# xuankuzcr/Global-LVBA

Hardware: NVIDIA H100
Metric: LM iterations/sec (Jacobian+Hessian build + Schur solve) (higher is better)
Workload: dtype f64

## Files before the change

global-lvba_b200/csrc/factor_la.cuh:

```cuda
#pragma once
#include "envelope.cuh"

namespace lvba {

constexpr bool la_tile2(int P) { return P > 24; }
constexpr int la_tile2_threads(int P) { int s = 0; for (int m = 1; m <= P; ++m) s += (m + 1) / 2; return s; }
template <int P, bool kTile2>
struct LaCfg {
  static constexpr int kPairs = P * (P + 1) / 2;
  static constexpr int kOwners = kTile2 ? la_tile2_threads(P) : kPairs;
  static constexpr bool kRealloc = P > 24;
  static constexpr int kPairThreads = kRealloc ? ((kOwners + 127) / 128) * 128 : ((kOwners + 31) / 32) * 32;
  static constexpr int kLaThreads = 128;
  static constexpr int kThreads = kPairThreads + kLaThreads;
  static constexpr int kItemThreads = 96;
  static constexpr int kItems = (P - 1) * 6;
  static constexpr int kRounds = (kItems + kItemThreads - 1) / kItemThreads;
  static constexpr int S = 38;
  static constexpr int kPairRegs = kTile2 ? 200 : 104, kLaRegs = kTile2 ? 96 : 64;
  static constexpr int kDoubles = 6 * P * S + 2 * P * 36 + 2 * 36 + 36 + 2 * 36 + P * 6 + 48 + 40 + 48;
  static constexpr size_t kSmem = sizeof(double) * (size_t)kDoubles + sizeof(long long) * 64 + sizeof(int) * 64 + 32;
};

LVBA_DEV void cp_async16_zfill(void* smem, const void* gmem, bool valid) {
// ... 474 lines not shown
          const int i = (l21 >= 15) ? 5 : (l21 >= 10) ? 4 : (l21 >= 6) ? 3 : (l21 >= 3) ? 2 : (l21 >= 1) ? 1 : 0;
          const int j = l21 - i * (i + 1) / 2;
          double v = dg[i * 6 + j];
          double w = 0.0;
#pragma unroll
          for (int q = 0; q < 6; q += 2) { v -= l1[q * 6 + i] * T1[q * 6 + j]; w += l1[(q + 1) * 6 + i] * T1[(q + 1) * 6 + j]; }
          v -= w;
          if (lane < 21) sDu[i * 6 + j] = v;
          __syncwarp();
          invert_pivot(sDu, sK + nxt * 36, k + 1);
        }
        named_bar_sync(1, Cfg::kLaThreads);
        double zk[6];
#pragma unroll
        for (int q = 0; q < 6; ++q) zk[q] = sZ[c * 6 + q];
        if (lane < 6) z[6 * (long long)k + lane] = sZ[c * 6 + lane];
        __syncwarp();
        if (lane + 1 < P) {
          int slot = c + 1 + lane; if (slot >= P) slot -= P;
          const double2* lt2 = reinterpret_cast<const double2*>(Lc + slot * S);
          double acc[6];
#pragma unroll
          for (int x = 0; x < 6; ++x) acc[x] = sZ[slot * 6 + x];
#pragma unroll
          for (int q = 0; q < 6; ++q) {
            const double2 l0 = lt2[3 * q], l1 = lt2[3 * q + 1], l2 = lt2[3 * q + 2];
            acc[0] -= l0.x * zk[q]; acc[1] -= l0.y * zk[q]; acc[2] -= l1.x * zk[q]; acc[3] -= l1.y * zk[q]; acc[4] -= l2.x * zk[q]; acc[5] -= l2.y * zk[q];
          }
#pragma unroll
          for (int x = 0; x < 6; ++x) sZ[slot * 6 + x] = acc[x];
        }
        __syncwarp();
        if (lane < 6) sZ[c * 6 + lane] = (k + P < n) ? sZin[((k + P) & 7) * 6 + lane] : 0.0;
        if (J.progress && lane == 0 && (k & 3) == 3) progress_publish(J.progress, k + 1);
      } else {
        stream_row(k + 1);
        if (it < 5) {
          const int rl = k + 40, rz = k + P + 4;
          if (it == 0 && rl < n) {
            asm volatile("cp.async.ca.shared.global [%0], [%1], 4;" ::"r"((unsigned)__cvta_generic_to_shared(sLabF + (rl & 63))), "l"(e.first + rl));
          } else if (it == 1 && rl < n) {
            asm volatile("cp.async.ca.shared.global [%0], [%1], 8;" ::"r"((unsigned)__cvta_generic_to_shared(sLabRS + (rl & 63))), "l"(e.row_start + rl));
          } else if (it >= 2 && rz < n) {
            cp_async16_zfill(sZin + (rz & 7) * 6 + 2 * (it - 2), z + 6 * (long long)rz + 2 * (it - 2), true);
          }
        }
        double t[Cfg::kRounds][6];
#pragma unroll
        for (int rd = 0; rd < Cfg::kRounds; ++rd) {
          const int slot = slot_[rd], x = x_[rd];
          if (ent_[rd]) {
            const double* en = sEnter + (cur * P) * 36 + x * 6;
#pragma unroll
            for (int q = 0; q < 6; ++q) t[rd][q] = en[q];
          } else {
            const double* as = sA + cur * PS + slot * S;
#pragma unroll
            for (int q = 0; q < 6; ++q) t[rd][q] = as[q * 6 + x];
            const double* lr = Lc + slot * S;
#pragma unroll
            for (int r = 0; r < 6; ++r) {
              const double lv = lr[r * 6 + x];
              const double2 u0 = reinterpret_cast<const double2*>(T1 + r * 6)[0];
              const double2 u1 = reinterpret_cast<const double2*>(T1 + r * 6)[1];
              const double2 u2 = reinterpret_cast<const double2*>(T1 + r * 6)[2];
              t[rd][0] -= lv * u0.x; t[rd][1] -= lv * u0.y; t[rd][2] -= lv * u1.x; t[rd][3] -= lv * u1.y; t[rd][4] -= lv * u2.x; t[rd][5] -= lv * u2.y;
            }
// ... 204 lines not shown
```

global-lvba_b200/csrc/nd_kernels.cuh:

```cuda
#pragma once
#include "envelope.cuh"
#include "factor_la.cuh"
#include "nd_passes.h"

namespace lvba {

template <class F>
__global__ void __launch_bounds__(256) nd_pass_kernel(long long n, F f) {
  for (long long i = (long long)blockIdx.x * blockDim.x + threadIdx.x; i < n; i += (long long)gridDim.x * blockDim.x) f(i);
}

constexpr int kSpikeC = 4;
constexpr int kSpikeWarps = 4;
constexpr int kSpikeCols = kSpikeC * kSpikeWarps;
constexpr int kSpikeThreads = 32 * kSpikeWarps;
constexpr int kSpikeZStride = 26;
constexpr int kSpikeBS = 38;
constexpr int kSpikeBufs = 3;
constexpr size_t kSpikeSmem = sizeof(double) * (kSpikeBufs * 32 * kSpikeBS + kSpikeWarps * 33 * kSpikeZStride);
static_assert(kSpikeC == 4, "the reduce-scatter below is written for 24 values per lane");

__global__ void __launch_bounds__(kSpikeThreads)
nd_spike_kernel(const nd::SpikeJob* __restrict__ jobs) {
  extern __shared__ __align__(16) double smem_spike[];
  double* sRow = smem_spike;
  const nd::SpikeJob J = jobs[blockIdx.y];
  const EnvView e = J.e;
  const int c0 = blockIdx.x * kSpikeCols;
  if (c0 >= J.KS) return;
  const int tid = threadIdx.x, lane = tid & 31, warp = tid >> 5;
  const int cw = c0 + warp * kSpikeC;
  double* sZw = smem_spike + kSpikeBufs * 32 * kSpikeBS + warp * 33 * kSpikeZStride;
  const int n = e.n, n_stop = J.n_stop, KS = J.KS;
  if (lane < kSpikeZStride) sZw[32 * kSpikeZStride + lane] = 0.0;
  for (int o = tid; o < kSpikeBufs * 32 * kSpikeBS; o += kSpikeThreads) sRow[o] = 0.0;
  const int sb0 = tid / 18, sh = tid - sb0 * 18;
  const int og = (lane >> 2) * 3;
  const bool owner = (lane & 3) == 0;
  int ox[3], oc[3];
#pragma unroll
  for (int q = 0; q < 3; ++q) { ox[q] = (og + q) >> 2; oc[q] = (og + q) & 3; }
  __syncthreads();
  auto stage_row = [&](int k, int f, long long rs) {
    if (k >= n) return;
    const int jend = k < n_stop ? k : n_stop;
    const int nb = jend > f ? jend - f : 0;
    const double* src = J.L + rs * 36;
    double* dst = sRow + (k % kSpikeBufs) * (32 * kSpikeBS);
    if (tid < 126)
      for (int b = sb0; b < nb; b += 7) cp_async16_zfill(dst + b * kSpikeBS + 2 * sh, src + b * 36 + 2 * sh, true);
  };
  int f0 = e.first[0];
  int f1 = n > 1 ? e.first[1] : 0; long long rs1 = n > 1 ? e.row_start[1] : 0;
  int f2 = n > 2 ? e.first[2] : 0; long long rs2 = n > 2 ? e.row_start[2] : 0;
  int f3 = n > 3 ? e.first[3] : 0; long long rs3 = n > 3 ? e.row_start[3] : 0;
  double en[3];
// ... 43 lines not shown
          double a = l[0] * z[c];
#pragma unroll
          for (int y = 1; y < 6; ++y) a = fma(l[y], z[y * 4 + c], a);
          v[x * 4 + c] = a;
        }
      }
    }
    const bool b16 = lane & 16, b8 = lane & 8, b4 = lane & 4;
    double w12[12], w6[6], w3[3];
#pragma unroll
    for (int o = 0; o < 12; ++o) {
      const double send = b16 ? v[o] : v[o + 12];
      const double keep = b16 ? v[o + 12] : v[o];
      w12[o] = keep + __shfl_xor_sync(0xffffffffu, send, 16);
    }
#pragma unroll
    for (int o = 0; o < 6; ++o) {
      const double send = b8 ? w12[o] : w12[o + 6];
      const double keep = b8 ? w12[o + 6] : w12[o];
      w6[o] = keep + __shfl_xor_sync(0xffffffffu, send, 8);
    }
#pragma unroll
    for (int o = 0; o < 3; ++o) {
      const double send = b4 ? w6[o] : w6[o + 3];
      const double keep = b4 ? w6[o + 3] : w6[o];
      w3[o] = keep + __shfl_xor_sync(0xffffffffu, send, 4);
    }
#pragma unroll
    for (int o = 0; o < 3; ++o) {
      w3[o] += __shfl_xor_sync(0xffffffffu, w3[o], 2);
      w3[o] += __shfl_xor_sync(0xffffffffu, w3[o], 1);
    }
    __syncwarp();
    if (owner) {
#pragma unroll
      for (int q = 0; q < 3; ++q) {
        const double r = ecur[q] - w3[q];
        sZw[(k & 31) * kSpikeZStride + ox[q] * 4 + oc[q]] = r;
        if (cw + oc[q] < KS) J.Z[((long long)k * 6 + ox[q]) * KS + cw + oc[q]] = r;
      }
    }
    __syncwarp();
    f0 = f1; f1 = f2; f2 = f3; rs2 = rs3; f3 = f4; rs3 = rs4;
  }
}

constexpr int kSyrkTile = 64;
constexpr int kSyrkThreads = 64;
constexpr int kSyrkChunk = 4;
constexpr int kSyrkSplit = 8;
constexpr int kSyrkLd = kSyrkTile + 4;
constexpr int kSyrkTileDoubles = kSyrkChunk * 6 * kSyrkLd;
constexpr size_t kSyrkSmem = sizeof(double) * (5 * kSyrkTileDoubles + 2 * kSyrkChunk * 36 + 2 * kSyrkChunk * 6 + kSyrkChunk * 6);

__global__ void __launch_bounds__(kSyrkThreads)
nd_syrk_kernel(const nd::SyrkSeg* __restrict__ segs, int split) {
  constexpr int TS = kSyrkTile, RC = kSyrkChunk * 6, LD = kSyrkLd;
  extern __shared__ __align__(16) double smem_syrk[];
  double* sA = smem_syrk;
  double* sB = sA + 2 * kSyrkTileDoubles;
  double* sY = sB + 2 * kSyrkTileDoubles;
  double* sK = sY + kSyrkTileDoubles;
  double* sW = sK + 2 * kSyrkChunk * 36;
  double* sKw = sW + 2 * RC;
  const nd::SyrkSeg G = segs[blockIdx.z];
  int ti = 0, tj = 0;
  { int t = blockIdx.x; while ((ti + 1) * (ti + 2) / 2 <= t) ++ti; tj = t - ti * (ti + 1) / 2; }
  if (ti * TS >= G.KS) return;
  const int k0 = blockIdx.y * split;
  if (k0 >= G.rows) return;
  const int k1 = min(G.rows, k0 + split);
  const int tid = threadIdx.x, tx = tid & 7, ty = tid >> 3;
  const int KS = G.KS;
  auto prefetch = [&](int kc, int par) {
    const int nr = min(kSyrkChunk, k1 - kc) * 6;
    double* dA = sA + par * kSyrkTileDoubles;
    double* dB = sB + par * kSyrkTileDoubles;
    for (int o = tid; o < RC * (TS / 2); o += kSyrkThreads) {
      const int r = o / (TS / 2), a2 = (o - r * (TS / 2)) * 2;
      const double* zr = G.Z + ((long long)kc * 6 + (r < nr ? r : 0)) * KS;
      const bool va = r < nr && ti * TS + a2 < KS, vb = r < nr && tj * TS + a2 < KS;
      cp_async16_zfill(dA + r * LD + a2, va ? zr + ti * TS + a2 : G.Z, va);
      cp_async16_zfill(dB + r * LD + a2, vb ? zr + tj * TS + a2 : G.Z, vb);
    }
    for (int o = tid; o < kSyrkChunk * 18; o += kSyrkThreads) {
      const int bk = o / 18;
      const bool v = kc + bk < k1;
      cp_async16_zfill(sK + par * kSyrkChunk * 36 + 2 * o, v ? G.K + (long long)kc * 36 + 2 * o : G.K, v);
    }
    for (int o = tid; o < kSyrkChunk * 3; o += kSyrkThreads) {
      const int bk = o / 3;
      const bool v = kc + bk < k1;
      cp_async16_zfill(sW + par * RC + 2 * o, v ? G.w + (long long)kc * 6 + 2 * o : G.w, v);
    }
  };
  double acc[8][8];
#pragma unroll
  for (int i = 0; i < 8; ++i)
#pragma unroll
    for (int j = 0; j < 8; ++j) acc[i][j] = 0.0;
  double racc = 0.0;
  prefetch(k0, 0);
  asm volatile("cp.async.commit_group;" ::: "memory");
  int par = 0;
  for (int kc = k0; kc < k1; kc += kSyrkChunk, par ^= 1) {
    if (kc + kSyrkChunk < k1) prefetch(kc + kSyrkChunk, par ^ 1);
    asm volatile("cp.async.commit_group;" ::: "memory");
    asm volatile("cp.async.wait_group 1;" ::: "memory");
    __syncthreads();
    const double* cA = sA + par * kSyrkTileDoubles;
    const double* cB = sB + par * kSyrkTileDoubles;
    const double* cK = sK + par * kSyrkChunk * 36;
    for (int o = tid; o < RC * TS; o += kSyrkThreads) {
      const int r = o / TS, b = o - r * TS, bk = r / 6, x = r - bk * 6;
      const double* Kx = cK + bk * 36 + x * 6;
      double s = 0.0;
#pragma unroll
      for (int q = 0; q < 6; ++q) s += Kx[q] * cB[(bk * 6 + q) * LD + b];
      sY[r * LD + b] = s;
    }
    if (tj == 0 && tid < RC) {
      const int bk = tid / 6, x = tid - bk * 6;
      double s = 0.0;
#pragma unroll
      for (int q = 0; q < 6; ++q) s += cK[bk * 36 + x * 6 + q] * sW[par * RC + bk * 6 + q];
      sKw[tid] = s;
    }
    __syncthreads();
#pragma unroll 2
    for (int r = 0; r < RC; ++r) {
      double av[8], bv[8];
#pragma unroll
      for (int m = 0; m < 4; ++m) {
        const double2 a = *reinterpret_cast<const double2*>(cA + r * LD + 2 * ty + 16 * m);
        const double2 b = *reinterpret_cast<const double2*>(sY + r * LD + 2 * tx + 16 * m);
        av[2 * m] = a.x; av[2 * m + 1] = a.y; bv[2 * m] = b.x; bv[2 * m + 1] = b.y;
      }
#pragma unroll
      for (int i = 0; i < 8; ++i)
#pragma unroll
        for (int j = 0; j < 8; ++j) acc[i][j] = fma(av[i], bv[j], acc[i][j]);
    }
    if (tj == 0 && tid < TS) {
      double s = 0.0;
      for (int r = 0; r < RC; ++r) s += cA[r * LD + tid] * sKw[r];
      racc += s;
    }
    __syncthreads();
  }
#pragma unroll
  for (int i = 0; i < 8; ++i)
#pragma unroll
    for (int j = 0; j < 8; ++j) {
      const int ga = ti * TS + 2 * ty + 16 * (i >> 1) + (i & 1), gb = tj * TS + 2 * tx + 16 * (j >> 1) + (j & 1);
      const int bi = ga / 6, bj = gb / 6;
      if (bj <= bi && ga < KS && gb < KS) atomicAdd(&G.U[((long long)bi * (bi + 1) / 2 + bj) * 36 + (ga - 6 * bi) * 6 + (gb - 6 * bj)], -acc[i][j]);
    }
  if (tj == 0 && tid < TS && ti * TS + tid < KS) atomicAdd(&G.u[ti * TS + tid], -racc);
}

__global__ void __launch_bounds__(192)
nd_correct_apply_kernel(nd::Tables t, const int* __restrict__ ids, int stride) {
  __shared__ double sc[6];
  const nd::NodeDev v = t.nodes[ids[blockIdx.x / stride]];
  const int k = blockIdx.x % stride;
  if (k >= v.npiv) return;
  const int tid = threadIdx.x, lane = tid & 31, q = tid >> 5;
  const double* wv = (v.kind == 0 ? t.z : t.zs) + 6 * (long long)(v.r0 + k);
  const double* zr = t.Z + v.offZ + ((long long)k * 6 + q) * v.ks;
  const int na = 6 * v.wa;
  const double* xa = t.x + 6 * (long long)v.sa;
  const double* xc = t.x + 6 * (long long)v.sc;
  double s = 0.0;
  for (int col = lane; col < v.ks; col += 32) s += zr[col] * (col < na ? xa[col] : xc[col - na]);
  s = warp_sum(s);
  if (lane == 0) sc[q] = wv[q] - s;
  __syncthreads();
  if (tid < 6) {
    const double* K = t.dinv + (long long)(v.r0 + k) * 36 + tid * 6;
    double o = 0.0;
#pragma unroll
    for (int qq = 0; qq < 6; ++qq) o += K[qq] * sc[qq];
// ... 55 lines not shown
        }
        if (i == s) {
          double2* d2 = reinterpret_cast<double2*>(sD + r * 6);
          d2[0] = make_double2(t[0], t[1]); d2[1] = make_double2(t[2], t[3]); d2[2] = make_double2(t[4], t[5]);
        }
      }
      if (!idle) {
        named_bar_sync(2, kDenseColThreads + 32);
        named_bar_sync(3, kDenseColThreads + 32);
      }
      if (mine && i > s) {
        double lr[6] = {0, 0, 0, 0, 0, 0};
        const double2* k2 = reinterpret_cast<const double2*>(sK + par * 36);
#pragma unroll
        for (int q = 0; q < 6; ++q) {
          const double2 k0 = k2[3 * q], k1 = k2[3 * q + 1], kk2 = k2[3 * q + 2];
          lr[0] = fma(t[q], k0.x, lr[0]); lr[1] = fma(t[q], k0.y, lr[1]); lr[2] = fma(t[q], k1.x, lr[2]);
          lr[3] = fma(t[q], k1.y, lr[3]); lr[4] = fma(t[q], kk2.x, lr[4]); lr[5] = fma(t[q], kk2.y, lr[5]);
        }
        double* tt = sT + (par * kDenseMax + i) * kDenseS + r;
        double* lt = sL + (par * kDenseMax + i) * kDenseS + r;
        double2* g2 = reinterpret_cast<double2*>(J.L + ((long long)i * (i + 1) / 2 + s) * 36 + r * 6);
#pragma unroll
        for (int q = 0; q < 6; ++q) { tt[q * 6] = t[q]; lt[q * 6] = lr[q]; }
#pragma unroll
        for (int h = 0; h < 3; ++h) g2[h] = make_double2(lr[2 * h], lr[2 * h + 1]);
        double zs = 0.0;
#pragma unroll
        for (int q = 0; q < 6; ++q) { zs = fma(lr[q], sZ[s * 6 + q], zs); lrow[q] = lr[q]; }
        sZ[i * 6 + r] -= zs;
      }
      __syncthreads();
      if (idle) {
        if (ct - kDenseColThreads < 18)
          reinterpret_cast<double2*>(J.dinv + (long long)s * 36)[ct - kDenseColThreads] = reinterpret_cast<const double2*>(sK + par * 36)[ct - kDenseColThreads];
        if (J.progress && ct == kDenseColThreads + 32 && (s & 3) == 3) progress_publish(J.progress, s + 1);
      }
    }
  } else if (tid >= kDenseInvWarp) {
    const int lane = tid - kDenseInvWarp;
    int bad = 0;
    __syncthreads();
    for (int s = 0; s < n; ++s) {
      named_bar_sync(2, kDenseColThreads + 32);
      double* Kp = sK + (s & 1) * 36;
      sym6_block_inverse_warp(sD, Kp, sInv, lane);
      __syncwarp();
      if (!isfinite((Kp[0] + Kp[35]) + (Kp[18] + Kp[13]))) bad = 1;
      named_bar_sync(3, kDenseColThreads + 32);
      __syncthreads();
    }
    if (bad && lane == 0) J.status[0] = 1;
  } else {
    const unsigned short tm = tmap[tid];
    const int i = tm & 0xff, j = tm >> 8;
    const bool live = tm != 0xffff && i < n;
    double G[36];
    if (live) {
      const double2* src = reinterpret_cast<const double2*>(J.L + ((long long)i * (i + 1) / 2 + j) * 36);
#pragma unroll
      for (int q = 0; q < 18; ++q) { const double2 v = src[q]; G[2 * q] = v.x; G[2 * q + 1] = v.y; }
    } else {
#pragma unroll
      for (int q = 0; q < 36; ++q) G[q] = 0.0;
    }
    auto publish = [&](int c) {
      double2* d2 = reinterpret_cast<double2*>(sC + ((c & 1) * kDenseMax + i) * kDenseS);
#pragma unroll
      for (int q = 0; q < 18; ++q) d2[q] = make_double2(G[2 * q], G[2 * q + 1]);
    };
    if (live && j <= 1) publish(j);
    __syncthreads();
    for (int s = 0; s < n; ++s) {
      if (s >= 1 && live && j >= s + 1) {
        const int par = (s - 1) & 1;
        const double2* l2 = reinterpret_cast<const double2*>(sL + (par * kDenseMax + i) * kDenseS);
        const double2* t2 = reinterpret_cast<const double2*>(sT + (par * kDenseMax + j) * kDenseS);
#pragma unroll
        for (int q = 0; q < 6; ++q) {
          const double2 t0 = t2[3 * q], t1 = t2[3 * q + 1], t2v = t2[3 * q + 2];
#pragma unroll
          for (int xp = 0; xp < 3; ++xp) {
            const double2 lv = l2[3 * q + xp];
            const double l0 = -lv.x, l1 = -lv.y;
            double* g0 = G + (2 * xp) * 6;
            double* g1 = G + (2 * xp + 1) * 6;
            g0[0] = fma(l0, t0.x, g0[0]); g0[1] = fma(l0, t0.y, g0[1]); g0[2] = fma(l0, t1.x, g0[2]);
            g0[3] = fma(l0, t1.y, g0[3]); g0[4] = fma(l0, t2v.x, g0[4]); g0[5] = fma(l0, t2v.y, g0[5]);
            g1[0] = fma(l1, t0.x, g1[0]); g1[1] = fma(l1, t0.y, g1[1]); g1[2] = fma(l1, t1.x, g1[2]);
            g1[3] = fma(l1, t1.y, g1[3]); g1[4] = fma(l1, t2v.x, g1[4]); g1[5] = fma(l1, t2v.y, g1[5]);
          }
        }
        if (j == s + 1) publish(s + 1);
      }
      __syncthreads();
    }
  }
  __syncthreads();
  for (int o = tid; o < n * 6; o += kDenseThreads) J.z[o] = sZ[o];
  if (J.progress) {
    __syncthreads();
    if (tid == 0) progress_publish(J.progress, n);
  }
}

inline std::vector<unsigned short> dense_thread_map() {
  struct B { int i, j; };
  std::vector<B> v;
  for (int i = 0; i < kDenseMax; ++i) for (int j = 0; j <= i; ++j) v.push_back(B{i, j});
  std::stable_sort(v.begin(), v.end(), [](const B& a, const B& b) {
    const int ka[4] = {a.i / 8, a.j / 4, a.i, a.j}, kb[4] = {b.i / 8, b.j / 4, b.i, b.j};
    for (int q = 0; q < 4; ++q) if (ka[q] != kb[q]) return ka[q] < kb[q];
    return false;
  });
  std::vector<unsigned short> m((size_t)kDensePairThreads, (unsigned short)0xffff);
  for (size_t t = 0; t < v.size(); ++t) m[t] = (unsigned short)(v[t].i | (v[t].j << 8));
  return m;
}

}
```

global-lvba_b200/csrc/nd_passes.h:

```cpp
#pragma once
#include <math.h>
#include <stdint.h>

#include "env_types.h"
#include "nd_plan.h"

#if defined(__CUDACC__)
#define LVBA_NHD __host__ __device__ __forceinline__
#else
#define LVBA_NHD inline
#endif

namespace lvba {
namespace nd {

struct NodeDev {
  int kind, r0, npiv, ntrail, sa, wa, sc, wc, left, right, ks, nE, nb, zrows;
  long long offU, offu, offZ, offE, offT, offW, offw;
};
inline NodeDev to_dev(const Node& v) {
  return NodeDev{v.kind, v.r0, v.npiv, v.ntrail, v.sa, v.wa, v.sc, v.wc, v.left, v.right, v.ks, v.nE, v.nb, v.zrows,
                 v.offU, v.offu, v.offZ, v.offE, v.offT, v.offW, v.offw};
}

struct SpikeJob {
  EnvView e;
  const double* L;
  int n_stop;
  const double* E;
  int nE;
  double* Z;
  int KS;
  const int* progress = nullptr;
};
struct SyrkSeg {
  const double* Z;
  const double* K;
  const double* w;
  int rows;
  int KS;
  double* U;
  double* u;
};

struct Tables {
  int n;
  const int* first;
  const long long* row_start;
  const NodeDev* nodes;
  const double* H;
  const double* dadd;
  double* L;
  double* z;
  double* zs;
  double* dinv;
  double* x;
  double* U; double* u; double* Z; double* E; double* T; double* W; double* w;
  double* Hw; double* daddw;
  int* prog = nullptr;
};

LVBA_NHD void tri_dec(long long t, int& a, int& b) {
  long long i = (long long)((sqrt(8.0 * (double)t + 1.0) - 1.0) * 0.5);
  while ((i + 1) * (i + 2) / 2 <= t) ++i;
  while (i * (i + 1) / 2 > t) --i;
  a = (int)i;
  b = (int)(t - i * (i + 1) / 2);
}
LVBA_NHD long long tri_off(int i, int j) { return ((long long)i * (i + 1) / 2 + j) * 36; }
LVBA_NHD double mat_elem(const Tables& t, int r, int c, int x, int y) {
  if (c < t.first[r]) return 0.0;
  const double* b = t.H + (t.row_start[r] + (c - t.first[r])) * 36;
  if (r == c) {
    const double v = (x >= y) ? b[x * 6 + y] : b[y * 6 + x];
    return (x == y) ? v + t.dadd[6 * r + x] : v;
  }
  return b[x * 6 + y];
}
LVBA_NHD double upd_elem(const double* U, int i, int j, int x, int y) {
  return (i >= j) ? U[tri_off(i, j) + x * 6 + y] : U[tri_off(j, i) + y * 6 + x];
}

struct AddDiagF {
  Tables t;
  LVBA_NHD void operator()(int64_t i) const {
    const int r = (int)(i / 6), a = (int)(i % 6);
    t.L[(t.row_start[r] + (r - t.first[r])) * 36 + a * 7] += t.dadd[i];
  }
};

struct LeafEF {
  Tables t; const int* ids; long long stride;
// ... 219 lines not shown

struct DenseViewArrays {
  const int* zeros;
  const long long* tri;
  const int* last_by_w;
};

inline void build_level_jobs(const Plan& P, const Tables& t, const int* first_rel, const long long* rs_adj, const int* last_rel,
                             long long nblocks, const DenseViewArrays& dv, int* status, std::vector<LevelJobs>& out, int my_rank = 0) {
  out.assign(P.levels.size(), LevelJobs());
  for (size_t lv = 0; lv < P.levels.size(); ++lv) {
    LevelJobs& J = out[lv];
    for (int id : P.levels[lv])
      if (P.nodes[id].owner < 0 || P.nodes[id].owner == my_rank) J.ids.push_back(id);
    for (int id : J.ids) {
      const Node& v = P.nodes[id];
      EnvView e;
      double* Lp;
      double* zp;
      if (v.kind == 0) {
        e = EnvView{v.npiv + v.ntrail, first_rel + v.r0, rs_adj + v.r0, last_rel + v.r0, nblocks};
        Lp = t.L; zp = t.z + 6 * (long long)v.r0;
        for (int r = v.r0; r < v.r0 + v.npiv + v.ntrail; ++r) J.max_col = std::max(J.max_col, r - v.r0 - P.first_rel[r]);
      } else {
        e = EnvView{v.npiv, dv.zeros, dv.tri, dv.last_by_w + v.npiv * 32, (long long)v.npiv * (v.npiv + 1) / 2};
        Lp = t.T + v.offT; zp = t.zs + 6 * (long long)v.r0;
        J.max_col = std::max(J.max_col, v.npiv - 1);
      }
      J.factor.push_back(FactorJob{e, Lp, t.dinv + 36 * (long long)v.r0, zp, v.npiv,
                                   v.ntrail ? t.W + v.offW : nullptr, v.ntrail ? t.w + v.offw : nullptr, status + id,
                                   (t.prog && v.ks > 0) ? t.prog + id : nullptr});
      J.back.push_back(BacksolveJob{e, Lp, t.x + 6 * (long long)v.r0, v.npiv});
      if (v.ks > 0) {
        J.spike.push_back(SpikeJob{e, Lp, v.npiv, t.E + v.offE, v.kind == 0 ? v.nE : v.npiv, t.Z + v.offZ, v.ks, t.prog ? t.prog + id : nullptr});
        J.syrk.push_back(SyrkSeg{t.Z + v.offZ, t.dinv + 36 * (long long)v.r0, zp, v.npiv, v.ks, t.U + v.offU, t.u + v.offu});
        J.max_ks = std::max(J.max_ks, v.ks);
      }
      J.max_rows = std::max(J.max_rows, v.npiv);
      J.corr_stride = std::max(J.corr_stride, v.npiv);
      if (v.kind == 1) J.asm_stride = std::max(J.asm_stride, sep_items(v));
    }
  }
}

struct LevelDev {
  const int* ids; int n_ids;
  const FactorJob* factor; int n_factor;
  const SpikeJob* spike; int n_spike;
  const SyrkSeg* syrk; int n_syrk;
  const BacksolveJob* back; int n_back;
  long long asm_stride; int corr_stride; int max_ks, max_rows, max_col;
};

template <class Exec>
inline void run_up_local(Exec& ex, const Plan& P, const Tables& t, const LevelDev* lv, int n_levels, long long nblocks,
                         long long leaf_e, long long leaf_fin, const RegionDev* reg) {
  ex.copy(t.L, t.H, nblocks * 36);
  if (t.prog) ex.pass((long long)P.nodes.size(), ZeroProgF{t.prog});
  ex.pass((long long)6 * t.n, AddDiagF{t});
  ex.zero(t.U, P.sizeU);
  const LevelDev& L0 = lv[0];
  if (L0.n_spike) ex.pass((long long)L0.n_ids * leaf_e, LeafEF{t, L0.ids, leaf_e});
  ex.factor(L0.factor, L0.n_factor, L0.max_col);
  if (L0.n_spike) {
    ex.spike(L0.spike, L0.n_spike, L0.max_ks, P.max_zrows_leaf);
    ex.syrk(L0.syrk, L0.n_syrk, L0.max_ks, L0.max_rows);
  }
  ex.pass((long long)L0.n_ids * leaf_fin, LeafFinalF{t, L0.ids, leaf_fin});
  const int n_local = P.n_ranks > 1 ? P.local_levels : n_levels;
  for (int l = 1; l < n_local; ++l) {
    const LevelDev& J = lv[l];
    if (J.n_ids == 0) continue;
    ex.pass((long long)J.n_ids * J.asm_stride, SepAssembleF{t, J.ids, J.asm_stride});
    ex.factor_dense(J.factor, J.n_factor, J.max_col);
    if (J.n_spike) {
      ex.spike(J.spike, J.n_spike, J.max_ks, J.max_rows);
      ex.syrk(J.syrk, J.n_syrk, J.max_ks, J.max_rows);
    }
  }
  if (P.n_ranks > 1 && reg) ex.pass(reg->slotH + (long long)reg->slot_rows * 6, PackF{t, *reg});
}

template <class Exec>
inline void run_top_down(Exec& ex, const Plan& P, const Tables& t, const LevelDev* lv, int n_levels, const RegionDev* reg) {
  if (P.n_ranks > 1 && reg) {
    ex.pass((long long)reg->n_ranks * (reg->slotH + (long long)reg->slot_rows * 6), UnpackF{t, *reg});
    for (int l = P.local_levels; l < n_levels; ++l) {
      const LevelDev& J = lv[l];
      if (J.n_ids == 0) continue;
      ex.pass((long long)J.n_ids * J.asm_stride, SepAssembleF{t, J.ids, J.asm_stride});
      ex.factor_dense(J.factor, J.n_factor, J.max_col);
// ... 24 lines not shown
```

global-lvba_b200/csrc/nd_solver.cuh:

```cuda
#pragma once
#include <functional>

#include "nd_kernels.cuh"

namespace lvba {

struct NdDevice {
  nd::Plan plan;
  bool ready = false;
  int chunks = 0;
  DevBuf<int> d_first_rel, d_last_rel, d_zeros, d_last_by_w, d_ids;
  DevBuf<long long> d_rs_adj, d_tri;
  DevBuf<nd::NodeDev> d_nodes;
  DevBuf<int> d_sep_row0, d_sep_rows;
  nd::RegionDev reg{};
  int n_ranks = 1, my_rank = 0;
  DevBuf<double> xchg;
  DevBuf<unsigned short> d_dense_map;
  DevBuf<int> d_prog;
  DevBuf<double> zs, U, u, Z, E, T, W, w;
  DevBuf<FactorJob> d_factor;
  DevBuf<nd::SpikeJob> d_spike;
  DevBuf<nd::SyrkSeg> d_syrk;
  DevBuf<BacksolveJob> d_back;
  std::vector<nd::LevelDev> lv;
  nd::Tables tab{};
  long long leaf_e = 1, leaf_fin = 1;
  const double* key_H = nullptr; const double* key_dadd = nullptr; const double* key_x = nullptr; const double* key_z = nullptr;
  cudaGraph_t graph = nullptr;
  cudaGraphExec_t graph_exec = nullptr;
  bool use_graph = true;
  int64_t launches_per_solve = 0;

  ~NdDevice() { drop_graph(); }
  void drop_graph() {
    if (graph_exec) { cudaGraphExecDestroy(graph_exec); graph_exec = nullptr; }
    if (graph) { cudaGraphDestroy(graph); graph = nullptr; }
  }

  static int default_chunks(int n, int max_col) {
    if (n < 768) return 0;
    const long long want = (long long)n / (3LL * max_col + 30);
    int best = 0;
    for (int p = 4; p <= 256 && p <= want; p *= 2) best = p;
    return best;
  }

  int prepare(int n, const std::vector<int>& first, const std::vector<int>& last, const std::vector<long long>& row_start, int max_col,
              int p_want, cudaStream_t s, int n_ranks_ = 1, int my_rank_ = 0) {
    ready = false; chunks = 0;
    drop_graph();
    key_H = key_dadd = key_x = key_z = nullptr;
    n_ranks = n_ranks_; my_rank = my_rank_;
    if (n_ranks > 1) p_want = std::max(n_ranks, ((p_want + n_ranks - 1) / n_ranks) * n_ranks);
    if (p_want < 2) return LVBA_OK;
    const int p = nd::choose_chunks(n, first.data(), last.data(), row_start.data(), max_col, p_want, plan, n_ranks);
    if (p < 2) return LVBA_OK;
    if (n_ranks > 1) {
      for (int r = 0; r < n_ranks; ++r)
        if (plan.rank_row_end[r] - plan.rank_row_begin[r] < max_col + 1) return LVBA_OK;
    }
    {
      const char* g = getenv("LVBA_ND_GRAPH");
      use_graph = !(g && g[0] == '0');
    }
    int64_t dummy = 0;
    LVBA_TRY(d_first_rel.upload(plan.first_rel, s, &dummy));
    LVBA_TRY(d_last_rel.upload(plan.last_rel, s, &dummy));
    LVBA_TRY(d_rs_adj.upload(plan.rs_adj, s, &dummy));
    std::vector<int> zeros(32, 0), last_by_w(32 * 32, 0);
    std::vector<long long> tri(33, 0);
    for (int i = 0; i < 33; ++i) tri[i] = (long long)i * (i + 1) / 2;
    for (int w_ = 0; w_ < 32; ++w_) for (int i = 0; i < 32; ++i) last_by_w[w_ * 32 + i] = w_ - 1;
    LVBA_TRY(d_zeros.upload(zeros, s, &dummy));
    LVBA_TRY(d_last_by_w.upload(last_by_w, s, &dummy));
    LVBA_TRY(d_tri.upload(tri, s, &dummy));
    std::vector<nd::NodeDev> nodes;
    for (const nd::Node& v : plan.nodes) nodes.push_back(nd::to_dev(v));
    LVBA_TRY(d_nodes.upload(nodes, s, &dummy));
    const std::vector<unsigned short> dmap = dense_thread_map();
    LVBA_TRY(d_dense_map.upload(dmap, s, &dummy));
    LVBA_TRY(zs.alloc((size_t)n * 6));
    LVBA_TRY(U.alloc((size_t)std::max<long long>(plan.sizeU, 1))); LVBA_TRY(u.alloc((size_t)std::max<long long>(plan.sizeu, 1)));
    LVBA_TRY(Z.alloc((size_t)std::max<long long>(plan.sizeZ, 1))); LVBA_TRY(E.alloc((size_t)std::max<long long>(plan.sizeE, 1)));
    LVBA_TRY(T.alloc((size_t)std::max<long long>(plan.sizeT, 1))); LVBA_TRY(W.alloc((size_t)std::max<long long>(plan.sizeW, 1)));
    LVBA_TRY(w.alloc((size_t)std::max<long long>(plan.sizew, 1)));
    if (n_ranks > 1) {
      std::vector<int> s0((size_t)n_ranks, -1), sr((size_t)n_ranks, 0);
      for (int r = 0; r + 1 < n_ranks; ++r) { s0[r] = plan.sep_start[(r + 1) * plan.q]; sr[r] = plan.sep_width[(r + 1) * plan.q]; }
      LVBA_TRY(d_sep_row0.upload(s0, s, &dummy)); LVBA_TRY(d_sep_rows.upload(sr, s, &dummy));
      reg = nd::RegionDev{n_ranks, my_rank, plan.slot_rows, plan.max_col, plan.region0, plan.slot, plan.slotU, plan.slotu, plan.slotH,
                          d_sep_row0.p, d_sep_rows.p};
      long long mx = 0;
      for (int r = 0; r < n_ranks; ++r) {
        const int b = plan.rank_row_begin[r], e2 = std::min(n, b + max_col);
        mx = std::max(mx, (row_start[e2] - row_start[b]) * 36);
      }
      LVBA_TRY(xchg.alloc((size_t)std::max<long long>(mx, 1)));
    }
    LVBA_TRY(d_prog.alloc(plan.nodes.size()));
    LVBA_CUDA(cudaFuncSetAttribute(nd_spike_kernel, cudaFuncAttributeMaxDynamicSharedMemorySize, (int)kSpikeSmem));
    LVBA_CUDA(cudaFuncSetAttribute(nd_syrk_kernel, cudaFuncAttributeMaxDynamicSharedMemorySize, (int)kSyrkSmem));
    LVBA_CUDA(cudaFuncSetAttribute(nd_dense_factor_kernel, cudaFuncAttributeMaxDynamicSharedMemorySize, (int)kDenseSmem));
    LVBA_CUDA(cudaStreamSynchronize(s));
    leaf_e = nd::leaf_e_stride(plan); leaf_fin = nd::leaf_final_stride(plan);
    chunks = p; ready = true;
    return LVBA_OK;
  }

  int build_tables(const EnvView& genv, const double* H, const double* dadd, double* L, double* dinv, double* z, double* x,
                   int* status, cudaStream_t s) {
    if (key_H == H && key_dadd == dadd && key_x == x && key_z == z && !lv.empty()) return LVBA_OK;
    drop_graph();
    tab = nd::Tables{};
    tab.n = plan.n; tab.first = genv.first; tab.row_start = genv.row_start; tab.nodes = d_nodes.p;
    tab.H = H; tab.dadd = dadd; tab.L = L; tab.z = z; tab.zs = zs.p; tab.dinv = dinv; tab.x = x;
    tab.U = U.p; tab.u = U.p; tab.Z = Z.p; tab.E = E.p; tab.T = T.p; tab.W = W.p; tab.w = w.p;
    tab.Hw = n_ranks > 1 ? const_cast<double*>(H) : nullptr;
    tab.daddw = n_ranks > 1 ? const_cast<double*>(dadd) : nullptr;
    tab.prog = d_prog.p;
    std::vector<nd::LevelJobs> jobs;
    nd::DenseViewArrays dv{d_zeros.p, d_tri.p, d_last_by_w.p};
    nd::build_level_jobs(plan, tab, d_first_rel.p, d_rs_adj.p, d_last_rel.p, genv.nblocks, dv, status + 1, jobs, my_rank);
    std::vector<int> ids; std::vector<FactorJob> fj; std::vector<nd::SpikeJob> sj; std::vector<nd::SyrkSeg> yj; std::vector<BacksolveJob> bj;
    struct Off { size_t ids, f, s, y, b; };
    std::vector<Off> off;
    for (auto& J : jobs) {
      off.push_back(Off{ids.size(), fj.size(), sj.size(), yj.size(), bj.size()});
      ids.insert(ids.end(), J.ids.begin(), J.ids.end());
      fj.insert(fj.end(), J.factor.begin(), J.factor.end());
      sj.insert(sj.end(), J.spike.begin(), J.spike.end());
      yj.insert(yj.end(), J.syrk.begin(), J.syrk.end());
      bj.insert(bj.end(), J.back.begin(), J.back.end());
    }
    LVBA_TRY(d_ids.upload(ids, s)); LVBA_TRY(d_factor.upload(fj, s)); LVBA_TRY(d_back.upload(bj, s));
    if (!sj.empty()) { LVBA_TRY(d_spike.upload(sj, s)); LVBA_TRY(d_syrk.upload(yj, s)); }
    LVBA_CUDA(cudaStreamSynchronize(s));
    lv.clear();
    for (size_t l = 0; l < jobs.size(); ++l) {
      const auto& J = jobs[l];
      lv.push_back(nd::LevelDev{d_ids.p + off[l].ids, (int)J.ids.size(), d_factor.p + off[l].f, (int)J.factor.size(),
                                d_spike.p + off[l].s, (int)J.spike.size(), d_syrk.p + off[l].y, (int)J.syrk.size(),
                                d_back.p + off[l].b, (int)J.back.size(), J.asm_stride, J.corr_stride, J.max_ks, J.max_rows, J.max_col});
    }
    key_H = H; key_dadd = dadd; key_x = x; key_z = z;
    return LVBA_OK;
  }
};

struct NdCudaExec {
  cudaStream_t s;
  std::function<int(int, int, const FactorJob*)> factor_fn;
  std::function<void(int, const BacksolveJob*)> back_fn;
// ... 3 lines not shown
  template <class F> void pass(long long n, const F& f) {
    if (n <= 0) return;
    const int grid = (int)std::min<long long>((n + 255) / 256, kNumSMs * 8);
    nd_pass_kernel<<<grid, 256, 0, s>>>(n, f);
    ++launches;
  }
  void copy(double* dst, const double* src, long long n) { cudaMemcpyAsync(dst, src, (size_t)n * sizeof(double), cudaMemcpyDeviceToDevice, s); }
  void zero(double* p, long long n) { if (n > 0) cudaMemsetAsync(p, 0, (size_t)n * sizeof(double), s); }
  void factor(const FactorJob* jobs, int n, int max_col) {
    if (n <= 0) return;
    const int r = factor_fn(max_col, n, jobs);
    if (r != LVBA_OK) rc = r;
  }
  void factor_dense(const FactorJob* jobs, int n, int max_col) {
    if (n <= 0) return;
    nd_dense_factor_kernel<<<n, kDenseThreads, kDenseSmem, s>>>(jobs, dense_map);
    ++launches;
  }
  void spike(const nd::SpikeJob* jobs, int n, int max_ks, int) {
    if (n <= 0 || max_ks <= 0) return;
    cudaLaunchConfig_t cfg = {};
    cfg.gridDim = dim3((max_ks + kSpikeCols - 1) / kSpikeCols, n); cfg.blockDim = dim3(kSpikeThreads); cfg.dynamicSmemBytes = kSpikeSmem; cfg.stream = s;
    cudaLaunchAttribute at[1];
    at[0].id = cudaLaunchAttributeProgrammaticStreamSerialization;
    at[0].val.programmaticStreamSerializationAllowed = 1;
    cfg.attrs = at; cfg.numAttrs = 1;
    const cudaError_t e = cudaLaunchKernelEx(&cfg, nd_spike_kernel, jobs);
    if (e != cudaSuccess) rc = fail(LVBA_ERR_CUDA, "cudaLaunchKernelEx(nd_spike_kernel): %s", cudaGetErrorString(e));
    ++launches;
  }
  void syrk(const nd::SyrkSeg* segs, int n, int max_ks, int max_rows) {
    if (n <= 0 || max_ks <= 0) return;
    const int nt1 = (max_ks + kSyrkTile - 1) / kSyrkTile, nt = nt1 * (nt1 + 1) / 2;
    nd_syrk_kernel<<<dim3(nt, (max_rows + kSyrkSplit - 1) / kSyrkSplit, n), kSyrkThreads, kSyrkSmem, s>>>(segs, kSyrkSplit);
    ++launches;
  }
  void correct_apply(const nd::Tables& t, const int* ids, int n_ids, int stride) {
    if (n_ids <= 0 || stride <= 0) return;
    nd_correct_apply_kernel<<<n_ids * stride, 192, 0, s>>>(t, ids, stride);
    ++launches;
  }
  void backsolve(const BacksolveJob* jobs, int n) {
    if (n <= 0) return;
    back_fn(n, jobs);
    ++launches;
  }
};

}
```

Before: 330.5.

## Overlap spike and SYRK kernels via per-column-group progress counters and PDL

The spike kernel now triggers programmatic dependent launch and publishes per-column-group row progress counters, and the SYRK kernel is launched with PDL and polls these counters (plus the factor progress) so it can start consuming Z rows before the spike finishes. SYRK single-buffers the B tile to save shared memory and handles partial chunks. The dense factor writes z rows incrementally instead of at the end, and the heuristic for the number of chunks changes to scale with sqrt(n). This aims to hide the serial gap between kernels, at the cost of spin-polling, more progress memory, and the risk of deadlock if the blocks are not co-resident.

```diff
diff --git a/global-lvba_b200/csrc/factor_la.cuh b/global-lvba_b200/csrc/factor_la.cuh
--- a/global-lvba_b200/csrc/factor_la.cuh
+++ b/global-lvba_b200/csrc/factor_la.cuh
@@ -530,7 +530,7 @@
         }
         __syncwarp();
         if (lane < 6) sZ[c * 6 + lane] = (k + P < n) ? sZin[((k + P) & 7) * 6 + lane] : 0.0;
-        if (J.progress && lane == 0 && (k & 3) == 3) progress_publish(J.progress, k + 1);
+        if (J.progress && lane == 0 && (k & 3) == 3 && k + 1 < n_stop) progress_publish(J.progress, k + 1);
       } else {
         stream_row(k + 1);
         if (it < 5) {
diff --git a/global-lvba_b200/csrc/nd_kernels.cuh b/global-lvba_b200/csrc/nd_kernels.cuh
--- a/global-lvba_b200/csrc/nd_kernels.cuh
+++ b/global-lvba_b200/csrc/nd_kernels.cuh
@@ -18,10 +18,12 @@
 constexpr int kSpikeBS = 38;
 constexpr int kSpikeBufs = 3;
 constexpr size_t kSpikeSmem = sizeof(double) * (kSpikeBufs * 32 * kSpikeBS + kSpikeWarps * 33 * kSpikeZStride);
+constexpr int kSpikePublish = 4;
 static_assert(kSpikeC == 4, "the reduce-scatter below is written for 24 values per lane");
 
 __global__ void __launch_bounds__(kSpikeThreads)
 nd_spike_kernel(const nd::SpikeJob* __restrict__ jobs) {
+  pdl_launch_dependents();
   extern __shared__ __align__(16) double smem_spike[];
   double* sRow = smem_spike;
   const nd::SpikeJob J = jobs[blockIdx.y];
@@ -131,6 +133,7 @@
       w3[o] += __shfl_xor_sync(0xffffffffu, w3[o], 1);
     }
     __syncwarp();
+    if (J.zprog && tid == 32 && k > 0 && k % kSpikePublish == 0) progress_publish(J.zprog + blockIdx.x, k);
     if (owner) {
 #pragma unroll
       for (int q = 0; q < 3; ++q) {
@@ -141,6 +144,11 @@
     }
     __syncwarp();
     f0 = f1; f1 = f2; f2 = f3; rs2 = rs3; f3 = f4; rs3 = rs4;
+  }
+  if (J.zprog) {
+    wait_row(n);
+    __syncthreads();
+    if (tid == 0) progress_publish(J.zprog + blockIdx.x, n);
   }
 }
 
@@ -150,7 +158,11 @@
 constexpr int kSyrkSplit = 8;
 constexpr int kSyrkLd = kSyrkTile + 4;
 constexpr int kSyrkTileDoubles = kSyrkChunk * 6 * kSyrkLd;
-constexpr size_t kSyrkSmem = sizeof(double) * (5 * kSyrkTileDoubles + 2 * kSyrkChunk * 36 + 2 * kSyrkChunk * 6 + kSyrkChunk * 6);
+constexpr size_t kSyrkSmem = sizeof(double) * (4 * kSyrkTileDoubles + 2 * kSyrkChunk * 36 + 2 * kSyrkChunk * 6 + kSyrkChunk * 6);
+constexpr int kSyrkTileGroups = kSyrkTile / kSpikeCols;
+static_assert(kSyrkTile % kSpikeCols == 0 && kSyrkChunk % kSpikePublish == 0 && kSyrkSplit % kSyrkChunk == 0,
+              "a chunk of the SYRK must end where the spike publishes");
+static_assert(2 * kSyrkTileGroups + 1 <= kSyrkThreads, "one polling thread per counter");
 
 __global__ void __launch_bounds__(kSyrkThreads)
 nd_syrk_kernel(const nd::SyrkSeg* __restrict__ segs, int split) {
@@ -158,29 +170,43 @@
   extern __shared__ __align__(16) double smem_syrk[];
   double* sA = smem_syrk;
   double* sB = sA + 2 * kSyrkTileDoubles;
-  double* sY = sB + 2 * kSyrkTileDoubles;
+  double* sY = sB + kSyrkTileDoubles;
   double* sK = sY + kSyrkTileDoubles;
   double* sW = sK + 2 * kSyrkChunk * 36;
   double* sKw = sW + 2 * RC;
-  const nd::SyrkSeg G = segs[blockIdx.z];
+  const nd::SyrkSeg G = segs[blockIdx.y];
   int ti = 0, tj = 0;
   { int t = blockIdx.x; while ((ti + 1) * (ti + 2) / 2 <= t) ++ti; tj = t - ti * (ti + 1) / 2; }
   if (ti * TS >= G.KS) return;
-  const int k0 = blockIdx.y * split;
+  const int k0 = blockIdx.z * split;
   if (k0 >= G.rows) return;
   const int k1 = min(G.rows, k0 + split);
   const int tid = threadIdx.x, tx = tid & 7, ty = tid >> 3;
   const int KS = G.KS;
+  const int* poll = nullptr;
+  if (G.zprog) {
+    if (tid < 2 * kSyrkTileGroups) {
+      const int g = (tid < kSyrkTileGroups ? ti : tj) * kSyrkTileGroups + tid % kSyrkTileGroups;
+      if (g * kSpikeCols < KS) poll = G.zprog + g;
+    } else if (tid == 2 * kSyrkTileGroups) {
+      poll = G.fprog;
+    }
+  }
+  auto need = [&](int r) { return poll == G.fprog ? min(r + 1, G.rows) : r; };
+  auto wait_rows = [&](int r) {
+    if (poll) { const int v = need(r); while (progress_read(poll) < v) __nanosleep(64); }
+  };
+  auto rows_ready = [&](int r) { return !poll || progress_read(poll) >= need(r); };
+  auto wait_spike_done = [&]() {
+    if (poll && tid < 2 * kSyrkTileGroups) while (progress_read(poll) < G.zdone) __nanosleep(64);
+  };
   auto prefetch = [&](int kc, int par) {
     const int nr = min(kSyrkChunk, k1 - kc) * 6;
     double* dA = sA + par * kSyrkTileDoubles;
-    double* dB = sB + par * kSyrkTileDoubles;
     for (int o = tid; o < RC * (TS / 2); o += kSyrkThreads) {
       const int r = o / (TS / 2), a2 = (o - r * (TS / 2)) * 2;
-      const double* zr = G.Z + ((long long)kc * 6 + (r < nr ? r : 0)) * KS;
-      const bool va = r < nr && ti * TS + a2 < KS, vb = r < nr && tj * TS + a2 < KS;
-      cp_async16_zfill(dA + r * LD + a2, va ? zr + ti * TS + a2 : G.Z, va);
-      cp_async16_zfill(dB + r * LD + a2, vb ? zr + tj * TS + a2 : G.Z, vb);
+      const bool va = r < nr && ti * TS + a2 < KS;
+      cp_async16_zfill(dA + r * LD + a2, va ? G.Z + ((long long)kc * 6 + r) * KS + ti * TS + a2 : G.Z, va);
     }
     for (int o = tid; o < kSyrkChunk * 18; o += kSyrkThreads) {
       const int bk = o / 18;
@@ -193,24 +219,38 @@
       cp_async16_zfill(sW + par * RC + 2 * o, v ? G.w + (long long)kc * 6 + 2 * o : G.w, v);
     }
   };
+  auto prefetch_col = [&](int kc) {
+    const int nr = min(kSyrkChunk, k1 - kc) * 6;
+    for (int o = tid; o < RC * (TS / 2); o += kSyrkThreads) {
+      const int r = o / (TS / 2), a2 = (o - r * (TS / 2)) * 2;
+      const bool vb = r < nr && tj * TS + a2 < KS;
+      cp_async16_zfill(sB + r * LD + a2, vb ? G.Z + ((long long)kc * 6 + r) * KS + tj * TS + a2 : G.Z, vb);
+    }
+  };
   double acc[8][8];
 #pragma unroll
   for (int i = 0; i < 8; ++i)
 #pragma unroll
     for (int j = 0; j < 8; ++j) acc[i][j] = 0.0;
   double racc = 0.0;
+  wait_rows(min(k0 + kSyrkChunk, k1));
+  __syncthreads();
   prefetch(k0, 0);
+  prefetch_col(k0);
   asm volatile("cp.async.commit_group;" ::: "memory");
   int par = 0;
   for (int kc = k0; kc < k1; kc += kSyrkChunk, par ^= 1) {
-    if (kc + kSyrkChunk < k1) prefetch(kc + kSyrkChunk, par ^ 1);
+    const int nr = min(kSyrkChunk, k1 - kc) * 6, next_r = min(kc + 2 * kSyrkChunk, k1);
+    const bool more = kc + kSyrkChunk < k1;
+    const bool early = more && __syncthreads_and(rows_ready(next_r));
+    if (early) prefetch(kc + kSyrkChunk, par ^ 1);
     asm volatile("cp.async.commit_group;" ::: "memory");
     asm volatile("cp.async.wait_group 1;" ::: "memory");
     __syncthreads();
     const double* cA = sA + par * kSyrkTileDoubles;
-    const double* cB = sB + par * kSyrkTileDoubles;
+    const double* cB = sB;
     const double* cK = sK + par * kSyrkChunk * 36;
-    for (int o = tid; o < RC * TS; o += kSyrkThreads) {
+    for (int o = tid; o < nr * TS; o += kSyrkThreads) {
       const int r = o / TS, b = o - r * TS, bk = r / 6, x = r - bk * 6;
       const double* Kx = cK + bk * 36 + x * 6;
       double s = 0.0;
@@ -218,7 +258,7 @@
       for (int q = 0; q < 6; ++q) s += Kx[q] * cB[(bk * 6 + q) * LD + b];
       sY[r * LD + b] = s;
     }
-    if (tj == 0 && tid < RC) {
+    if (tj == 0 && tid < nr) {
       const int bk = tid / 6, x = tid - bk * 6;
       double s = 0.0;
 #pragma unroll
@@ -226,8 +266,10 @@
       sKw[tid] = s;
     }
     __syncthreads();
+    if (early) prefetch_col(kc + kSyrkChunk);
+    asm volatile("cp.async.commit_group;" ::: "memory");
 #pragma unroll 2
-    for (int r = 0; r < RC; ++r) {
+    for (int r = 0; r < nr; ++r) {
       double av[8], bv[8];
 #pragma unroll
       for (int m = 0; m < 4; ++m) {
@@ -242,11 +284,18 @@
     }
     if (tj == 0 && tid < TS) {
       double s = 0.0;
-      for (int r = 0; r < RC; ++r) s += cA[r * LD + tid] * sKw[r];
+      for (int r = 0; r < nr; ++r) s += cA[r * LD + tid] * sKw[r];
       racc += s;
     }
-    __syncthreads();
+    if (more && !early) wait_rows(next_r);
+    __syncthreads();
+    if (more && !early) {
+      prefetch(kc + kSyrkChunk, par ^ 1);
+      prefetch_col(kc + kSyrkChunk);
+      asm volatile("cp.async.commit_group;" ::: "memory");
+    }
   }
+  if (k1 == G.rows) wait_spike_done();
 #pragma unroll
   for (int i = 0; i < 8; ++i)
 #pragma unroll
@@ -368,9 +417,12 @@
       }
       __syncthreads();
       if (idle) {
-        if (ct - kDenseColThreads < 18)
-          reinterpret_cast<double2*>(J.dinv + (long long)s * 36)[ct - kDenseColThreads] = reinterpret_cast<const double2*>(sK + par * 36)[ct - kDenseColThreads];
-        if (J.progress && ct == kDenseColThreads + 32 && (s & 3) == 3) progress_publish(J.progress, s + 1);
+        const int l = ct - kDenseColThreads;
+        if (l < 18)
+          reinterpret_cast<double2*>(J.dinv + (long long)s * 36)[l] = reinterpret_cast<const double2*>(sK + par * 36)[l];
+        else if (l < 24)
+          J.z[s * 6 + l - 18] = sZ[s * 6 + l - 18];
+        if (J.progress && l == 32 && (s & 3) == 3 && s + 1 < n) progress_publish(J.progress, s + 1);
       }
     }
   } else if (tid >= kDenseInvWarp) {
@@ -433,11 +485,7 @@
     }
   }
   __syncthreads();
-  for (int o = tid; o < n * 6; o += kDenseThreads) J.z[o] = sZ[o];
-  if (J.progress) {
-    __syncthreads();
-    if (tid == 0) progress_publish(J.progress, n);
-  }
+  if (J.progress && tid == 0) progress_publish(J.progress, n);
 }
 
 inline std::vector<unsigned short> dense_thread_map() {
diff --git a/global-lvba_b200/csrc/nd_passes.h b/global-lvba_b200/csrc/nd_passes.h
--- a/global-lvba_b200/csrc/nd_passes.h
+++ b/global-lvba_b200/csrc/nd_passes.h
@@ -32,6 +32,7 @@
   double* Z;
   int KS;
   const int* progress = nullptr;
+  int* zprog = nullptr;
 };
 struct SyrkSeg {
   const double* Z;
@@ -41,6 +42,9 @@
   int KS;
   double* U;
   double* u;
+  const int* fprog = nullptr;
+  const int* zprog = nullptr;
+  int zdone = 0;
 };
 
 struct Tables {
@@ -58,6 +62,7 @@
   double* U; double* u; double* Z; double* E; double* T; double* W; double* w;
   double* Hw; double* daddw;
   int* prog = nullptr;
+  int zstride = 0;
 };
 
 LVBA_NHD void tri_dec(long long t, int& a, int& b) {
@@ -343,8 +348,11 @@
                                    (t.prog && v.ks > 0) ? t.prog + id : nullptr});
       J.back.push_back(BacksolveJob{e, Lp, t.x + 6 * (long long)v.r0, v.npiv});
       if (v.ks > 0) {
-        J.spike.push_back(SpikeJob{e, Lp, v.npiv, t.E + v.offE, v.kind == 0 ? v.nE : v.npiv, t.Z + v.offZ, v.ks, t.prog ? t.prog + id : nullptr});
-        J.syrk.push_back(SyrkSeg{t.Z + v.offZ, t.dinv + 36 * (long long)v.r0, zp, v.npiv, v.ks, t.U + v.offU, t.u + v.offu});
+        int* zprog = t.prog ? t.prog + (long long)P.nodes.size() + (long long)id * t.zstride : nullptr;
+        J.spike.push_back(SpikeJob{e, Lp, v.npiv, t.E + v.offE, v.kind == 0 ? v.nE : v.npiv, t.Z + v.offZ, v.ks, t.prog ? t.prog + id : nullptr,
+                                   zprog});
+        J.syrk.push_back(SyrkSeg{t.Z + v.offZ, t.dinv + 36 * (long long)v.r0, zp, v.npiv, v.ks, t.U + v.offU, t.u + v.offu,
+                                 t.prog ? t.prog + id : nullptr, zprog, e.n});
         J.max_ks = std::max(J.max_ks, v.ks);
       }
       J.max_rows = std::max(J.max_rows, v.npiv);
@@ -367,7 +375,7 @@
 inline void run_up_local(Exec& ex, const Plan& P, const Tables& t, const LevelDev* lv, int n_levels, long long nblocks,
                          long long leaf_e, long long leaf_fin, const RegionDev* reg) {
   ex.copy(t.L, t.H, nblocks * 36);
-  if (t.prog) ex.pass((long long)P.nodes.size(), ZeroProgF{t.prog});
+  if (t.prog) ex.pass((long long)P.nodes.size() * (1 + t.zstride), ZeroProgF{t.prog});
   ex.pass((long long)6 * t.n, AddDiagF{t});
   ex.zero(t.U, P.sizeU);
   const LevelDev& L0 = lv[0];
diff --git a/global-lvba_b200/csrc/nd_solver.cuh b/global-lvba_b200/csrc/nd_solver.cuh
--- a/global-lvba_b200/csrc/nd_solver.cuh
+++ b/global-lvba_b200/csrc/nd_solver.cuh
@@ -18,6 +18,7 @@
   DevBuf<double> xchg;
   DevBuf<unsigned short> d_dense_map;
   DevBuf<int> d_prog;
+  int zstride = 0;
   DevBuf<double> zs, U, u, Z, E, T, W, w;
   DevBuf<FactorJob> d_factor;
   DevBuf<nd::SpikeJob> d_spike;
@@ -40,7 +41,7 @@
 
   static int default_chunks(int n, int max_col) {
     if (n < 768) return 0;
-    const long long want = (long long)n / (3LL * max_col + 30);
+    const double want = 16.0 * sqrt((double)n) / max_col;
     int best = 0;
     for (int p = 4; p <= 256 && p <= want; p *= 2) best = p;
     return best;
@@ -98,7 +99,9 @@
       }
       LVBA_TRY(xchg.alloc((size_t)std::max<long long>(mx, 1)));
     }
-    LVBA_TRY(d_prog.alloc(plan.nodes.size()));
+    zstride = 0;
+    for (const nd::Node& v : plan.nodes) zstride = std::max(zstride, (v.ks + kSpikeCols - 1) / kSpikeCols);
+    LVBA_TRY(d_prog.alloc(plan.nodes.size() * (size_t)(1 + zstride)));
     LVBA_CUDA(cudaFuncSetAttribute(nd_spike_kernel, cudaFuncAttributeMaxDynamicSharedMemorySize, (int)kSpikeSmem));
     LVBA_CUDA(cudaFuncSetAttribute(nd_syrk_kernel, cudaFuncAttributeMaxDynamicSharedMemorySize, (int)kSyrkSmem));
     LVBA_CUDA(cudaFuncSetAttribute(nd_dense_factor_kernel, cudaFuncAttributeMaxDynamicSharedMemorySize, (int)kDenseSmem));
@@ -118,7 +121,7 @@
     tab.U = U.p; tab.u = U.p; tab.Z = Z.p; tab.E = E.p; tab.T = T.p; tab.W = W.p; tab.w = w.p;
     tab.Hw = n_ranks > 1 ? const_cast<double*>(H) : nullptr;
     tab.daddw = n_ranks > 1 ? const_cast<double*>(dadd) : nullptr;
-    tab.prog = d_prog.p;
+    tab.prog = d_prog.p; tab.zstride = zstride;
     std::vector<nd::LevelJobs> jobs;
     nd::DenseViewArrays dv{d_zeros.p, d_tri.p, d_last_by_w.p};
     nd::build_level_jobs(plan, tab, d_first_rel.p, d_rs_adj.p, d_last_rel.p, genv.nblocks, dv, status + 1, jobs, my_rank);
@@ -188,7 +191,15 @@
   void syrk(const nd::SyrkSeg* segs, int n, int max_ks, int max_rows) {
     if (n <= 0 || max_ks <= 0) return;
     const int nt1 = (max_ks + kSyrkTile - 1) / kSyrkTile, nt = nt1 * (nt1 + 1) / 2;
-    nd_syrk_kernel<<<dim3(nt, (max_rows + kSyrkSplit - 1) / kSyrkSplit, n), kSyrkThreads, kSyrkSmem, s>>>(segs, kSyrkSplit);
+    cudaLaunchConfig_t cfg = {};
+    cfg.gridDim = dim3(nt, n, (max_rows + kSyrkSplit - 1) / kSyrkSplit); cfg.blockDim = dim3(kSyrkThreads); cfg.dynamicSmemBytes = kSyrkSmem;
+    cfg.stream = s;
+    cudaLaunchAttribute at[1];
+    at[0].id = cudaLaunchAttributeProgrammaticStreamSerialization;
+    at[0].val.programmaticStreamSerializationAllowed = 1;
+    cfg.attrs = at; cfg.numAttrs = 1;
+    const cudaError_t e = cudaLaunchKernelEx(&cfg, nd_syrk_kernel, segs, kSyrkSplit);
+    if (e != cudaSuccess) rc = fail(LVBA_ERR_CUDA, "cudaLaunchKernelEx(nd_syrk_kernel): %s", cudaGetErrorString(e));
     ++launches;
   }
   void correct_apply(const nd::Tables& t, const int* ids, int n_ids, int stride) {
```

Result: faster. 348.3, median of 6 (+5.4%).
